# huangjuite/form

Measured on AMD Instinct MI355X. Metric: scans/sec + Mpts/sec scan-to-submap ICP (128-beam); ATE delta vs reference, higher is better.
Workload: dtype fp32 points / fp64 map, residuals and normal equations; 1 GPU; c4: 128x2048 organized scan stream (262144 pts/scan), register_scan, smoothing mode (ConstraintManager default); parallelism=replicas x1, prefill=90, pipelined_extraction=True

## Files before the change

__graft_entry__.py:

```python
from __future__ import annotations

import os
import subprocess
import sys

ROOT = os.path.dirname(os.path.abspath(__file__))


def build() -> None:
    jobs = str(min(8, os.cpu_count() or 4))
    subprocess.check_call(["make", "-s", "-j", jobs, "-C", os.path.join(ROOT, "form_amd", "csrc")])
    subprocess.check_call(["make", "-s", "-C", os.path.join(ROOT, "oracle")])
    subprocess.check_call(["make", "-s", "-C", os.path.join(ROOT, "tests", "cpp")])
    if os.path.exists(os.path.join(ROOT, "tests", "cpp", "extract_plan.mk")):
        subprocess.check_call(["make", "-s", "-C", os.path.join(ROOT, "tests", "cpp"), "-f", "extract_plan.mk"])
    if os.path.exists(os.path.join(ROOT, "tests", "cpp", "carve_host.mk")):
        subprocess.check_call(["make", "-s", "-C", os.path.join(ROOT, "tests", "cpp"), "-f", "carve_host.mk"])
    if os.path.exists(os.path.join(ROOT, "tests", "cpp", "probe_host.mk")):
        subprocess.check_call(["make", "-s", "-C", os.path.join(ROOT, "tests", "cpp"), "-f", "probe_host.mk"])
    if os.path.exists(os.path.join(ROOT, "tests", "cpp", "scan_check.mk")):
        subprocess.check_call(["make", "-s", "-C", os.path.join(ROOT, "tests", "cpp"), "-f", "scan_check.mk"])
    if os.path.exists(os.path.join(ROOT, "tests", "cpp", "upload_host.mk")):
        subprocess.check_call(["make", "-s", "-C", os.path.join(ROOT, "tests", "cpp"), "-f", "upload_host.mk"])
    if os.path.exists(os.path.join(ROOT, "tests", "cpp", "nearest_host.mk")):
        subprocess.check_call(["make", "-s", "-C", os.path.join(ROOT, "tests", "cpp"), "-f", "nearest_host.mk"])
    if os.path.exists(os.path.join(ROOT, "tests", "cpp", "align_host.mk")):
        subprocess.check_call(["make", "-s", "-C", os.path.join(ROOT, "tests", "cpp"), "-f", "align_host.mk"])
    if os.path.exists(os.path.join(ROOT, "tests", "cpp", "store_plan.mk")):
        subprocess.check_call(["make", "-s", "-C", os.path.join(ROOT, "tests", "cpp"), "-f", "store_plan.mk"])
    sys.path.insert(0, ROOT)
    import form_amd
    from form_amd import fmx
    L = fmx.lib()
    missing = [s for s in fmx.EXPORTED if not hasattr(L, s)]
    if missing:
        raise RuntimeError(f"libfmx.so is missing symbols: {missing}")


def smoke() -> None:
    import numpy as np
    import torch

    sys.path.insert(0, ROOT)
    sys.path.insert(0, os.path.join(ROOT, "oracle"))
    import oracle_py as O

    from form_amd import fmx, synth

    assert torch.cuda.is_available(), "smoke() needs a GPU"
    scan, T, geo = synth.make_scan("tiny", 0)
    p = synth.default_params(geo)
    ref = O.extract(scan.numpy(), p)
    ctx = fmx.Context(fmx.EstimatorParams(extraction=fmx.KeypointExtractionParams(**p)))
    ctx.extract(scan.to("cuda:0"), 0)
    got = ctx.extract_download()
    ok = ref["normal_ok"]
    assert np.array_equal(got["planar_index"], ref["sel"][ok]), "planar selection differs from oracle"
    assert np.array_equal(got["point_index"], ref["point_idx"]), "point selection differs from oracle"
    dots = np.abs(np.sum(got["planar"][:, 3:] * ref["normals"][ok], 1))
    assert dots.min() > 1 - 1e-5, f"normals differ (min |dot| {dots.min()})"
    est = fmx.Context(fmx.EstimatorParams(extraction=fmx.KeypointExtractionParams(**p)))
    oest = O.Estimator(O.default_params(p))
    world = synth.World()
    for k in range(3):
        s, _, _ = synth.make_scan("tiny", k, world=world)
        est.register_scan(s.to("cuda:0"))
        Tg = est.current_pose()
        To, _, _ = oest.register_scan(s.numpy())
        assert np.abs(Tg - To).max() < 1e-6, f"scan {k}: pose differs from oracle by {np.abs(Tg - To).max()}"
    print("smoke ok:", len(got["planar_index"]), "planar,", len(got["point_index"]), "point; 3-scan registration matches oracle")


if __name__ == "__main__":
    build()
    if len(sys.argv) > 1 and sys.argv[1] == "smoke":
        smoke()
```

form_amd/csrc/fmx_api.cpp:

```cpp
#include <algorithm>
#include <atomic>
#include <cfloat>
#include <cmath>
#include <cstdlib>
#include <cstring>
#include <deque>
#include <functional>
#include <unistd.h>
#include <map>
#include <new>
#include <set>
#include <vector>

#include "fmx_api.hpp"

using namespace fmx;

namespace fmx {

int match_group_for(uint64_t nq, uint32_t K) { return (int)match_group(nq, K); }
void run_map_build(fmx_ctx* c, const std::vector<uint64_t>& scans, const double* poses34, double w, hipStream_t st) {
  ++c->warm_gen;
  g8::run_map_build(c, scans, poses34, w, st);
}
void run_match(fmx_ctx* c, const double* pose_j34, double max_dist, double min_dist_map, bool sorted,
               bool defer_scatter) {
  HostScope hs(16);
  ++c->corr_gen;
  c->m.match_group = match_group_for((uint64_t)c->n_qpl + c->n_qpt, c->K);
  if (c->m.match_group != 8) gl::run_match(c, pose_j34, max_dist, min_dist_map, sorted, defer_scatter);
  else g8::run_match(c, pose_j34, max_dist, min_dist_map, sorted, defer_scatter);
}
void run_pair_scatter(fmx_ctx* c) {
  HostScope hs(17);
  if (c->m.match_group != 8) gl::run_pair_scatter(c);
  else g8::run_pair_scatter(c);
}
void run_insert(fmx_ctx* c, uint64_t scan, uint32_t* n_inserted) {
  if (c->m.match_group != 8) gl::run_insert(c, scan, n_inserted);
  else g8::run_insert(c, scan, n_inserted);
}
void run_match_linearize(fmx_ctx* c, const double* pose_j34, double max_dist, double sigma, double* dst,
                         uint32_t* flag, uint32_t seq) {
  if (match_group_for((uint64_t)c->n_qpl + c->n_qpt, c->K) != 1)
    throw StatusError(FMX_E_STATE, "fused match + linearization needs the one-lane-per-query build");
  gl::run_match_linearize(c, pose_j34, max_dist, sigma, dst, flag, seq);
}
void match_counts_fetch(fmx_ctx* c, bool wait) {
  if (c->m.match_group != 8) gl::match_counts_fetch(c, wait);
  else g8::match_counts_fetch(c, wait);
}

static const char* kProfNames[PROF_COUNT] = {"extract_rows", "closest",   "fit",       "compact", "map_build",
                                             "match",        "pair_sort", "linearize", "insert",  "window",
                                             "match_linearize", "unpack", "moments", "deskew",
                                             "organize", "dense", "carve"};

ProfScope::ProfScope(Prof& p, int i, double by, hipStream_t s) : pr(p), id(i), bytes(by), st(s) {
  if (!pr.on) return;
  auto get = [&]() {
    hipEvent_t e;
    if (!pr.free_events.empty()) {
      e = pr.free_events.back();
      pr.free_events.pop_back();
    } else {
      FMX_HIP(hipEventCreate(&e));
    }
    return e;
  };
  a = get();
  b = get();
  FMX_HIP(hipEventRecord(a, st));
}
ProfScope::~ProfScope() {
  if (!a) return;
  (void)hipEventRecord(b, st);
  ProfPending e;
  e.id = id;
  e.a = a;
  e.b = b;
  e.bytes = bytes;
// ... 642 lines not shown
  c->spec_valid = true;
  c->spec_first = first;
  if (!first) ++c->spec_launched;
}
bool use_spec_match(fmx_ctx* c, const double* pose_j) {
  if (!c->spec_valid || std::memcmp(c->spec_pose, pose_j, sizeof(c->spec_pose)) != 0) return false;
  swap_match_set(c);
  c->spec_valid = false;
  if (!c->spec_first) ++c->spec_hits;
  c->spec_first = false;
  return true;
}

void keyscan_step(fmx_ctx* c, fmx_ctx::Est& e, uint64_t j, uint32_t nfeat);
void record_cons(fmx_ctx* c, fmx_ctx::Est& e, uint64_t j);

bool trace_on() {
  static const bool v = std::getenv("FMX_TRACE") != nullptr;
  return v;
}
#define FMX_TRACE_(...)                   \
  do {                                    \
    if (trace_on()) {                     \
      fprintf(stderr, __VA_ARGS__);       \
      fflush(stderr);                     \
    }                                     \
  } while (0)

bool lin_rows() {
  static const bool v = std::getenv("FMX_MOMENTS") == nullptr;
  return v;
}

void smooth_register(fmx_ctx* c, fmx_ctx::Est& e, uint64_t j, uint32_t nfeat, const LinF& fast, uint64_t& icp,
                     uint64_t& lm_it, uint64_t& lins, bool& inserted) {
  const fmx_params& P = c->P;
  const double sigma = P.planar_constraint_sigma;
  const std::vector<uint64_t> keys = window_keys(e);
  std::map<uint64_t, int> slot;
  for (size_t k = 0; k < keys.size(); ++k) slot[keys[k]] = (int)k;
  WinGraph g;
  g.keys = keys;
  for (auto& p : e.priors) g.priors.push_back(&p);
  for (auto& m : e.margs) g.lins.push_back(&m);
  if (!fast.keys.empty()) g.lins.push_back(&fast);
  std::vector<double> table;
  const bool mom = !lin_rows();
  const bool mom_full = mom;
  std::vector<double> momv;
  std::vector<Pose> mref;
  std::vector<const double*> mp;
  std::vector<const Pose*> mri, mrj, mxi, mxj;
  MomBatch mbatch;
  for (uint32_t it = 0; it < P.max_num_rematches; ++it) {
    ++icp;
    const Pose before = e.values.at(j);
    const bool spec_hit = use_spec_match(c, before.m);
    if (!spec_hit) run_match(c, before.m, P.max_dist_matching, P.min_dist_map, true);
    c->spec_valid = false;
    const bool mom_queued = spec_hit && c->spec_mom;
    c->spec_mom = false;
    pf_launch(c, false);
    g.pairs.clear();
    for (uint32_t k = 0; k < c->K; ++k) g.pairs.push_back({slot.at(c->map_scans[k]), slot.at(j)});
    const int K = (int)c->K;
    auto maybe_spec = [&](const std::vector<Pose>& x) {
      const Pose& xj = x[slot.at(j)];
      const double lc = g.trial_lin_change, ce = g.trial_err;
      bool last_likely = lc >= 0.0 && (lc <= 1e-5 * ce || lc <= 1e-5);
      if (last_likely) {
        double xi[6], dn = 0;
        logmap(compose(inverse(before), xj), xi);
        for (double v : xi) dn += v * v;
        last_likely = std::sqrt(dn) >= P.new_pose_threshold;
      }
      if (last_likely && it + 1 < P.max_num_rematches && std::memcmp(xj.m, before.m, sizeof(xj.m)) != 0) {
        FMX_TRACE_("  spec match\n");
        if (mom) {
          std::vector<double> ref(12 * ((size_t)K + 1));
          for (int k = 0; k < K; ++k) std::memcpy(&ref[12 * k], e.values.at(c->map_scans[k]).m, 12 * sizeof(double));
          std::memcpy(&ref[12 * (size_t)K], xj.m, 12 * sizeof(double));
          spec_match(c, xj.m, false, ref.data());
        } else {
          spec_match(c, xj.m);
        }
      }
    };
    bool launched = false, ready = false;
    int nlin = 0;
    if (mom) {
      auto lin_begin = [&](const std::vector<Pose>& x) {
        HostScope hs(10);
        if (!launched && mom_queued) {
          mref.resize((size_t)K + 1);
          for (int k = 0; k <= K; ++k) std::memcpy(mref[k].m, &c->spec_mom_ref[12 * (size_t)k], 12 * sizeof(double));
          momv.resize((size_t)std::max(K, 1) * kMomPairD);
          launched = true;
          FMX_TRACE_("scan %llu it %u: moments queued with the spec match\n", (unsigned long long)j, it);
        }
        if (!launched) {
          mref.resize((size_t)K + 1);
          table.resize(12 * ((size_t)K + 1));
          for (int k = 0; k < K; ++k) mref[k] = x[slot.at(c->map_scans[k])];
          mref[K] = x[slot.at(j)];
          for (int k = 0; k <= K; ++k) std::memcpy(&table[12 * k], mref[k].m, 12 * sizeof(double));
          momv.resize((size_t)std::max(K, 1) * kMomPairD);
          FMX_TRACE_("scan %llu it %u: moments launch K %d chunks %u\n", (unsigned long long)j, it, K, c->m.max_chunks);
          win_moments_current(c, table.data(), nullptr);
          FMX_TRACE_("  launched\n");
          launched = true;
        }
        maybe_spec(x);
        mxi.resize(K);
        mxj.resize(K);
        for (int k = 0; k < K; ++k) {
          mxi[k] = &x[slot.at(c->map_scans[k])];
          mxj[k] = &x[slot.at(j)];
        }
      };
      auto lin_end = [&](double* G) {
        HostScope hs(10);
        if (!ready) {
          FMX_TRACE_("  wait\n");
          win_finish(c, momv.data());
          FMX_TRACE_("  moments in\n");
          match_counts_fetch(c, false);
          for (int k = 0; k < K; ++k)
            if (c->m.cnt_pl[k] + c->m.cnt_pt[k] == 0)
              std::fill(&momv[(size_t)k * kMomPairD], &momv[(size_t)(k + 1) * kMomPairD], 0.0);
          mp.resize(K);
          mri.resize(K);
          mrj.assign(K, &mref[K]);
          for (int k = 0; k < K; ++k) {
            mp[k] = &momv[(size_t)k * kMomPairD];
            mri[k] = &mref[k];
          }
          HostScope hp(19);
          mom_prepare(mbatch, K, mp.data(), mri.data(), mrj.data());
          FMX_TRACE_("  prepared\n");
          ready = true;
        }
        HostScope he(18);
        mom_eval(mbatch, mxi.data(), mxj.data(), 1.0 / sigma, G);
        FMX_TRACE_("  eval\n");
      };
      set_lin(g, lin_begin, lin_end);
    } else {
      auto lin_begin = [&](const std::vector<Pose>& x) {
        table.resize(12 * ((size_t)K + 1));
        for (int k = 0; k < K; ++k) std::memcpy(&table[12 * k], x[slot.at(c->map_scans[k])].m, 12 * sizeof(double));
        std::memcpy(&table[12 * (size_t)K], x[slot.at(j)].m, 12 * sizeof(double));
        HostScope hs(10);
        win_linearize_current(c, table.data(), sigma, nullptr, nlin++ == 0 ? nullptr : c->lin);
        maybe_spec(x);
      };
      auto lin_end = [&](double* G) {
        HostScope hs(10);
        win_finish(c, G);
        match_counts_fetch(c, false);
        for (int k = 0; k < K; ++k)
          if (c->m.cnt_pl[k] + c->m.cnt_pt[k] == 0) std::fill(G + (size_t)k * kPairG, G + (size_t)(k + 1) * kPairG, 0.0);
      };
      set_lin(g, lin_begin, lin_end);
    }
    HostScope* hs_lm = new HostScope(8);
    FMX_TRACE_("scan %llu it %u: lm\n", (unsigned long long)j, it);
    const WinLMResult R = window_lm(g, window_poses(e));
    FMX_TRACE_("scan %llu it %u: lm done\n", (unsigned long long)j, it);
    delete hs_lm;
    lm_it += R.iters;
    lins += R.lins;
    const Pose after = R.x[slot.at(j)];
    double xi[6];
    logmap(compose(inverse(before), after), xi);
    double dn = 0;
    for (double v : xi) dn += v * v;
    if (std::sqrt(dn) < P.new_pose_threshold) break;
    e.values[j] = after;
  }
  record_cons(c, e, j);
  if (mom_full) {
    for (uint32_t k = 0; k < c->K; ++k)
      if (c->m.cnt_pl[k] + c->m.cnt_pt[k] > 0) {
        fmx_ctx::Est::Mom& m = e.moms[{j, c->map_scans[k]}];
        m.ref_i = mref[k];
        m.ref_j = mref[c->K];
        m.phi.assign(momv.begin() + (size_t)k * kMomPairD, momv.begin() + (size_t)(k + 1) * kMomPairD);
      }
  } else {
    win_persist(c, j);
  }
  ensure_pool_room(c, 0, c->n_qpl);
  ensure_pool_room(c, 1, c->n_qpt);
  run_insert(c, j, nullptr);
  inserted = true;
  keyscan_step(c, e, j, nfeat);
  c->ev_fork.record(c->stream);
  std::vector<uint64_t> map_scans;
  {
    std::set<uint64_t> sset;
    for (int t = 0; t < 2; ++t)
      for (auto& [s, r] : c->pool[t].ranges) sset.insert(s);
    map_scans.assign(sset.begin(), sset.end());
  }
  int spec_builds = 0;
  pf_launch(c, false);
  std::vector<WinPair> prs;
  if (mom_full) {
    for (auto& [ji, m] : e.moms) prs.push_back(WinPair{ji.second, ji.first, 0, 0, 0, 0});
  } else {
    prs = win_pairs(c);
  }
  g.lins.clear();
  for (auto& m : e.margs) g.lins.push_back(&m);
  g.pairs.clear();
  for (auto& p : prs) g.pairs.push_back({slot.at(p.i), slot.at(p.j)});
  if (!prs.empty() && !mom_full) win_set_pairs(c, prs, keys);
  auto maybe_spec_map = [&](const std::vector<Pose>& x) {
    const double lc = g.trial_lin_change, ce = g.trial_err;
    if (lc >= 0.0 && (lc <= 1e-5 * ce || lc <= 1e-5) && spec_builds < 2 && !map_scans.empty()) {
      ++spec_builds;
      std::vector<double> mpo(12 * map_scans.size());
      for (size_t k = 0; k < map_scans.size(); ++k) std::memcpy(&mpo[12 * k], x[slot.at(map_scans[k])].m, 12 * sizeof(double));
      FMX_TRACE_("  spec map (drain %d)\n", (int)e.spec_map);
      if (e.spec_map) FMX_HIP(hipStreamSynchronize(c->side));
      FMX_HIP(hipStreamWaitEvent(c->side, c->ev_fork.last(), 0));
      FMX_TRACE_("  spec map build\n");
      run_map_build(c, map_scans, mpo.data(), P.max_dist_matching, c->side);
      c->ev_join.record(c->side);
      FMX_TRACE_("  spec map queued\n");
      e.spec_map = true;
      e.spec_map_scans = map_scans;
      e.spec_map_poses = std::move(mpo);
    }
  };
  if (mom_full) {
    const size_t np = prs.size();
    mp.resize(np);
    mri.resize(np);
    mrj.resize(np);
    mxi.resize(np);
    mxj.resize(np);
    for (size_t p = 0; p < np; ++p) {
      const fmx_ctx::Est::Mom& m = e.moms.at({prs[p].j, prs[p].i});
      mp[p] = m.phi.data();
      mri[p] = &m.ref_i;
      mrj[p] = &m.ref_j;
    }
    {
      HostScope hp(19);
      mom_prepare(mbatch, (int)np, mp.data(), mri.data(), mrj.data());
    }
    g.lin_begin = nullptr;
    g.lin_end = nullptr;
    g.lin_pairs = [&, np](const std::vector<Pose>& x, double* G) {
      HostScope hs(10);
      FMX_TRACE_("  full lm lin (lin change %.3e)\n", g.trial_lin_change);
      maybe_spec_map(x);
      for (size_t p = 0; p < np; ++p) {
        mxi[p] = &x[g.pairs[p].first];
        mxj[p] = &x[g.pairs[p].second];
      }
      HostScope he(18);
      mom_eval(mbatch, mxi.data(), mxj.data(), 1.0 / sigma, G);
    };
  } else {
    auto lin_begin = [&](const std::vector<Pose>& x) {
      table.resize(12 * keys.size());
      for (size_t k = 0; k < keys.size(); ++k) std::memcpy(&table[12 * k], x[k].m, 12 * sizeof(double));
      HostScope hs(10);
// ... 241 lines not shown
    bool host_done = false;
    std::function<void()> host_first;
    if (c->dsk.on)
      host_first = [&] {
        map_inputs();
        finish();
        host_done = true;
      };
    if (pf_take(c, xyzw, n, on_dev, j, &fc, c->dsk.on ? &host_first : nullptr)) {
      if (c->dsk.on) {
        std::memcpy(dsk_xi, c->dsk.pf_twist, sizeof(dsk_xi));
        dsk_src = c->dsk.pf_src;
      }
      took_pf = true;
      if (!host_done) map_inputs();
      FMX_HIP(hipStreamWaitEvent(c->stream, c->ev_join.last(), 0));
      if (!P.disable_smoothing) {
        if (!lin_rows()) {
          std::vector<double> ref(12 * ((size_t)c->K + 1));
          for (uint32_t k = 0; k < c->K; ++k) std::memcpy(&ref[12 * k], e.values.at(c->map_scans[k]).m, 12 * sizeof(double));
          std::memcpy(&ref[12 * (size_t)c->K], e.values.at(j).m, 12 * sizeof(double));
          spec_match(c, e.values.at(j).m, true, ref.data());
        } else {
          spec_match(c, e.values.at(j).m, true);
        }
      }
      if (!host_done) finish();
    } else {
      do_extract(c, xyzw, n, j, on_dev, &fc, [&] {
        map_inputs();
        finish();
      }, c->dsk.on ? dsk_xi : nullptr, dsk_cells);
    }
  }
  std::memcpy(c->dsk.last, dsk_xi, sizeof(dsk_xi));
  c->dsk.last_src = dsk_src;
  const float4* dense_src = nullptr;
  if (dense_go) {
    if (c->dsk.on) {
      dense_src = took_pf ? c->dsk.pf_out.p : c->dsk.out.p;
    } else if (took_pf && c->pf_host) {
      DM.keep.ensure(n);
      FMX_HIP(hipMemcpyAsync(DM.keep.p, c->pf_scan.p, n * sizeof(float4), hipMemcpyDeviceToDevice, c->stream));
      dense_src = DM.keep.p;
    } else {
      dense_src = on_dev ? reinterpret_cast<const float4*>(xyzw) : c->scan.p;
    }
  }
  FMX_HIP(hipStreamWaitEvent(c->stream, c->ev_join.last(), 0));
  FMX_TRACE_("scan %llu: extracted %u + %u, map queued\n", (unsigned long long)j, fc.planar, fc.point);
  HostScope* hs_icp = new HostScope(4);
  uint64_t icp = 0, lm_it = 0, lins = 0;
  bool inserted = false;
  if (!P.disable_smoothing) {
    smooth_register(c, e, j, fc.planar + fc.point, fast, icp, lm_it, lins, inserted);
  } else {
    DeviceLM lm{c, e, P.planar_constraint_sigma};
    bool converged = false;
    Pose last_after = e.values.at(j);
    for (uint32_t it = 0; it < P.max_num_rematches; ++it) {
      ++icp;
      const Pose before = e.values.at(j);
      run_match(c, before.m, P.max_dist_matching, P.min_dist_map, false);
      pf_launch(c, false);
      int li = 0;
      const Pose after = lm.optimize(before, &li);
      lm_it += li;
      double xi[6];
      logmap(compose(inverse(before), after), xi);
      double dn = 0;
      for (double x : xi) dn += x * x;
      if (std::sqrt(dn) < P.new_pose_threshold) {
        converged = true;
        last_after = after;
        break;
      }
      e.values[j] = after;
    }
    if (converged) {
      e.values[j] = last_after;
    } else {
      int li = 0;
      e.values[j] = lm.optimize(e.values.at(j), &li);
      lm_it += li;
    }
    lins = lm.linearizations;
  }
  delete hs_icp;
  pf_launch(c, true);
  if (!inserted) {
    HostScope hs_tail(5);
    record_cons(c, e, j);
    ensure_pool_room(c, 0, c->n_qpl);
    ensure_pool_room(c, 1, c->n_qpt);
    run_insert(c, j, nullptr);
    keyscan_step(c, e, j, fc.planar + fc.point);
  }
  uint32_t dense_flag = 0;
  if (dense_go) dense_flag = dense_queue(c, dense_src, n, e.values.at(j).m, j);
  if (c->dsk.on && c->ann_ptr && !c->pf_launched) {
    double nxt[6];
    const int src = deskew_next_twist(c, nxt);
    pf_launch(c, true, nxt, src);
  }
  if (dense_go) {
    dense_finish(c, dense_flag, &DM.last);
// ... 46 lines not shown
  p->max_num_keyscans = 50;
  p->max_steps_unused_keyscan = 10;
  p->max_num_recent_scans = 10;
  p->keyscan_match_ratio = 0.1;
  p->min_dist_map = 0.1;
  p->keypoint_pool_capacity = 4u << 20;
  p->max_pairs = 1024;
  p->voxel_subdivision = 1;
}


fmx_status fmx_create(const fmx_params* p, int device, fmx_ctx** out) {
  if (!p || !out) return FMX_E_INVAL;
  *out = nullptr;
  int ndev = 0;
  if (hipGetDeviceCount(&ndev) != hipSuccess || ndev == 0) return FMX_E_HIP;
  if (device < 0 || device >= ndev) return FMX_E_INVAL;
  fmx_ctx* c = new (std::nothrow) fmx_ctx();
  if (!c) return FMX_E_OOM;
  c->P = *p;
  c->device = device;
  fmx_status st = guard(c, [&] {
    int prio_lo = 0, prio_hi = 0;
    FMX_HIP(hipDeviceGetStreamPriorityRange(&prio_lo, &prio_hi));
    FMX_HIP(hipStreamCreateWithPriority(&c->stream, hipStreamNonBlocking, prio_hi));
    FMX_HIP(hipStreamCreateWithPriority(&c->lin, hipStreamNonBlocking, prio_hi));
    {
      static std::atomic<uint32_t> ctx_seq{0};
      hipDeviceProp_t pr;
      FMX_HIP(hipGetDeviceProperties(&pr, device));
      const char* cus = std::getenv("FMX_SIDE_CUS");
      const int ncu = pr.multiProcessorCount, n = cus ? std::min(ncu, std::atoi(cus)) : std::max(1, ncu / 4);
      std::vector<uint32_t> m((ncu + 31) / 32, 0u);
      if (n <= 0) {
        std::fill(m.begin(), m.end(), 0xFFFFFFFFu);
      } else {
        const int q = (int)(ctx_seq.fetch_add(1u) % (uint32_t)std::max(1, ncu / n));
        for (int i = ncu - n * (q + 1); i < ncu - n * q; ++i) m[i / 32] |= 1u << (i % 32);
      }
      FMX_HIP(hipExtStreamCreateWithCUMask(&c->side, (uint32_t)m.size(), m.data()));
      FMX_HIP(hipExtStreamCreateWithCUMask(&c->side2, (uint32_t)m.size(), m.data()));
    }
    c->ev_fork.create();
    c->ev_join.create();
    c->ev_pf.create();
    c->ev_pf_fork.create();
    const uint64_t cap = p->keypoint_pool_capacity ? p->keypoint_pool_capacity : (4u << 20);
    c->pool[0].planar = true;
    c->pool[1].planar = false;
    c->pool[0].pos.ensure(cap);
    c->pool[0].nrm.ensure(cap);
    c->pool[1].pos.ensure(cap);
    c->store_limits = parse_store_limits(std::getenv("FMX_TEST_STORE_LIMITS"));
    for (int t = 0; t < 2; ++t) {
      const uint64_t alloc = c->pool[t].pos.cap;
      c->pool[t].limit = c->store_limits.pool ? std::min<uint64_t>(c->store_limits.pool, alloc) : alloc;
    }
  });
  if (st != FMX_OK) {
    fmx_destroy(c);
    return st;
  }
  *out = c;
  return FMX_OK;
}

fmx_ctx::~fmx_ctx() {
  for (hipStream_t s : {stream, side, side2, lin})
    if (s) (void)hipStreamSynchronize(s);
  stager.stop();
  delete est;
  comm_destroy(this);
  for (hipStream_t s : {stream, side, side2, lin})
    if (s) (void)hipStreamDestroy(s);
}

void fmx_destroy(fmx_ctx* c) {
  if (!c) return;
  (void)hipSetDevice(c->device);
  delete c;
}

const char* fmx_last_error(const fmx_ctx* c) { return c ? c->err.c_str() : "null context"; }

fmx_status fmx_extract(fmx_ctx* c, const float* xyzw, size_t n, uint64_t scan, int on_dev, fmx_feature_counts* out) {
  return guard<false>(c, [&] {
    drop_match(c);
    do_extract(c, xyzw, n, scan, on_dev, out);
  });
}

fmx_status fmx_extract_download(fmx_ctx* c, float* planar, uint32_t* planar_index, float* point,
                                uint32_t* point_index, uint8_t* planar_mask) {
  return guard(c, [&] {
    if (!c->have_queries) throw StatusError(FMX_E_STATE, "no extraction");
    FMX_HIP(hipStreamSynchronize(c->stream));
    const uint32_t npl = c->n_qpl, npt = c->n_qpt;
    if (planar) {
      std::vector<float4> a(npl), b(npl);
      FMX_HIP(hipMemcpy(a.data(), c->q.pl_pos.p, npl * sizeof(float4), hipMemcpyDeviceToHost));
      FMX_HIP(hipMemcpy(b.data(), c->q.pl_nrm.p, npl * sizeof(float4), hipMemcpyDeviceToHost));
      for (uint32_t i = 0; i < npl; ++i) {
        planar[6 * i] = a[i].x; planar[6 * i + 1] = a[i].y; planar[6 * i + 2] = a[i].z;
        planar[6 * i + 3] = b[i].x; planar[6 * i + 4] = b[i].y; planar[6 * i + 5] = b[i].z;
      }
    }
// ... 676 lines not shown
  return guard(c, [&] {
    if (!c->est || !c->est->init) throw StatusError(FMX_E_STATE, "no registered scan (fmx_register_scan)");
    if (!(voxel_width > 0)) throw StatusError(FMX_E_INVAL, "voxel width must be > 0");
    if (!n_planar || !n_point) throw StatusError(FMX_E_INVAL, "null count pointers");
    finish_tail(c);
    fmx_ctx::Est& e = *c->est;
    std::set<uint64_t> sset;
    for (int t = 0; t < 2; ++t)
      for (auto& [s, r] : c->pool[t].ranges) sset.insert(s);
    std::vector<uint64_t> scans(sset.begin(), sset.end());
    std::vector<double> poses(12 * scans.size());
    for (size_t k = 0; k < scans.size(); ++k) {
      auto it = e.values.find(scans[k]);
      if (it == e.values.end()) throw StatusError(FMX_E_STATE, "keypoints of a scan without an estimate");
      std::memcpy(&poses[12 * k], it->second.m, 12 * sizeof(double));
    }
    uint32_t cnt[2] = {0, 0};
    for (int t = 0; t < 2; ++t)
      for (uint64_t s : scans) {
        auto it = c->pool[t].ranges.find(s);
        if (it != c->pool[t].ranges.end()) cnt[t] += it->second.second;
      }
    double* outs[2] = {planar, point};
    uint64_t* sids[2] = {planar_scan, point_scan};
    uint32_t* ns[2] = {n_planar, n_point};
    for (int t = 0; t < 2; ++t) {
      if (!outs[t] && !sids[t]) {
        *ns[t] = cnt[t];
        continue;
      }
      if (*ns[t] < cnt[t]) throw StatusError(FMX_E_SIZE, "map_download: buffer smaller than the map");
      std::vector<double> xyz, nrm;
      std::vector<uint64_t> sid;
      const uint32_t m = map_snapshot(c, t, scans, poses, voxel_width, xyz, nrm, sid);
      const int stride = t == 0 ? 6 : 3;
      for (uint32_t r = 0; r < m; ++r) {
        if (outs[t]) {
          std::memcpy(outs[t] + (size_t)stride * r, &xyz[3 * (size_t)r], 3 * sizeof(double));
          if (t == 0) std::memcpy(outs[t] + (size_t)stride * r + 3, &nrm[3 * (size_t)r], 3 * sizeof(double));
        }
        if (sids[t]) sids[t][r] = sid[r];
      }
      *ns[t] = m;
    }
  });
}

fmx_status fmx_last_stats(fmx_ctx* c, uint64_t* stats, int n) {
  return guard<false>(c, [&] {
    if (!stats || n < 0) throw StatusError(FMX_E_INVAL, "null stats");
    const uint64_t store[kStatsStoreN] = {c->pool[0].n_compact, c->pool[1].n_compact, c->win.n_compact,
                                          c->win.n_grow_pl, c->win.n_grow_pt};
    for (int k = 0; k < n; ++k)
      stats[k] = k < kStatsN ? c->stats[k] : k < kStatsN + kStatsStoreN ? store[k - kStatsN] : 0;
  });
}

fmx_status fmx_match_work(fmx_ctx* c, double work[3]) {
  return guard<false>(c, [&] {
    match_counts_fetch(c);
    work[0] = (double)c->n_qpl + (double)c->n_qpt;
    work[1] = c->m.last_probes;
    work[2] = c->m.last_cands;
  });
}

fmx_status fmx_match_cert(fmx_ctx* c, uint64_t counts[2], uint8_t* certified) {
  return guard(c, [&] {
    if (!c->m.have_match) throw StatusError(FMX_E_STATE, "no match results");
    match_counts_fetch(c);
    if (counts) {
      counts[0] = c->m.cert_tot[0];
      counts[1] = c->m.cert_tot[1];
    }
    if (certified) {
      const uint32_t nq = c->n_qpl + c->n_qpt;
      std::vector<uint8_t> f(nq);
      if (nq) FMX_HIP(hipMemcpy(f.data(), c->m.m_ins.p, nq, hipMemcpyDeviceToHost));
      for (uint32_t q = 0; q < nq; ++q) certified[q] = (f[q] >> 1) & 1;
    }
  });
}

fmx_status fmx_profile_match_work(fmx_ctx* c, double out[12]) {
  return guard<false>(c, [&] {
    if (!out) throw StatusError(FMX_E_INVAL, "null output");
    prof_collect(c);
    for (int k = 0; k < 2; ++k)
      for (int i = 0; i < 6; ++i) out[6 * k + i] = c->prof.mwork[k][i];
  });
}

fmx_status fmx_corr_generation(fmx_ctx* c, uint64_t* gen) {
  return guard<false>(c, [&] {
    if (!gen) throw StatusError(FMX_E_INVAL, "null output");
    *gen = c->corr_gen;
  });
}

fmx_status fmx_profile_enable(fmx_ctx* c, int on) {
  return guard<false>(c, [&] { c->prof.on = on != 0; });
}
fmx_status fmx_profile_reset(fmx_ctx* c) {
  return guard<false>(c, [&] {
    prof_collect(c);
    for (int i = 0; i < PROF_COUNT; ++i) {
      c->prof.ms[i] = 0;
// ... 24 lines not shown
```

form_amd/csrc/fmx_internal.hpp:

```cpp
#pragma once
#include <hip/hip_runtime.h>

#include <atomic>
#include <stdint.h>

#include <algorithm>
#include <map>
#include <stdexcept>
#include <chrono>
#include <cstdio>
#include <cstdlib>
#include <functional>
#include <string>
#include <type_traits>
#include <utility>
#include <vector>

#include "fmx/fmx.h"
#include "carve_host.hpp"
#include "pair_sort_plan.hpp"
#include "probe_host.hpp"
#include "nearest_host.hpp"
#include "align_host.hpp"
#include "upload_host.hpp"
// ... 311 lines not shown
  int cur = 0;
  uint64_t cap_pl = 0, cap_pt = 0, tail_pl = 0, tail_pt = 0;
  WinSegs segs;
  bool exact_pl = false, exact_pt = false;
  uint64_t n_compact = 0, n_grow_pl = 0, n_grow_pt = 0;
  DBuf<uint32_t> meta;
  const Chunk* chunks_p = nullptr;
  const uint32_t* chunk_range_p = nullptr;
  Event meta_ev;
  bool meta_ev_pending = false;
  uint32_t nch = 0;
  int npairs = 0;
  uint64_t rows_pl = 0, rows_pt = 0;
  bool chunks_valid = false;
  DBuf<double> partials, dposes;
  DBuf<uint64_t> dbg;
  DBuf<uint32_t> pticket, dticket, dflag;
  bool pending = false;
  bool pending_mom = false;
  uint32_t pending_seq = 0, pending_grid = 0;
  hipStream_t pending_st = nullptr;
  int pending_np = 0;
  HBuf<double> hG, hM, hposes;
  HBuf<uint32_t> hmeta;
};

struct MatchSet {
  DBuf<int32_t> m_pair;
  DBuf<double> m_d2;
  DBuf<double4> m_pi, m_ni;
  DBuf<uint8_t> m_ins;
  DBuf<uint32_t> hist, hist_off;
  DBuf<uint32_t> thist;
  uint32_t thist_par = 0;
  DBuf<double> c_pl, c_pt;
  DBuf<uint32_t> pair_counts;
  DBuf<uint32_t> chunk_range;
  DBuf<Chunk> chunks;
  DBuf<uint32_t> n_chunks;
  DBuf<uint32_t> pair_base;
  DBuf<uint32_t> work;
  DBuf<uint32_t> mcnt, mticket;
  DBuf<uint32_t> ins_blk, ins_off;
  HBuf<uint32_t> h_counts, h_work;
  bool have_match = false, have_corr = false, have_qo = false;
  bool scatter_pending = false;
  bool counts_pending = false;
  size_t ld_pl = 0, ld_pt = 0;
  uint32_t max_chunks = 0, work_blocks = 0;
  uint32_t match_nb_pl = 0, match_nb = 0;
  uint32_t n_qo = 0;
  bool work_copied = false;
  int match_group = 8;
  PairScatter ps;
  uint64_t rows_pl = 0, rows_pt = 0;
  std::vector<uint32_t> cnt_pl, cnt_pt;
  double last_probes = 0, last_cands = 0;
  uint32_t ins_tot[2] = {0, 0};
  uint32_t cert_tot[2] = {0, 0};
};

struct QuerySet {
  DBuf<float4> pl_pos, pl_nrm, pt_pos;
  DBuf<uint32_t> pl_idx, pt_idx;
  DBuf<uint8_t> planar_mask;
};

struct ExLaunch {
  uint32_t seq = 0;
  const volatile uint32_t* flag = nullptr;
  const uint32_t* tot = nullptr;
  size_t max_pl = 0, max_pt = 0;
  hipStream_t st = nullptr;
};

}

constexpr int kStatsN = 14;
constexpr int kStatsStoreN = 5;

struct fmx_ctx {
  fmx_ctx() = default;
  fmx_ctx(const fmx_ctx&) = delete;
  fmx_ctx& operator=(const fmx_ctx&) = delete;
  ~fmx_ctx();

  fmx_params P{};
  int device = 0;
  hipStream_t stream = nullptr;
  hipStream_t side = nullptr;
  hipStream_t side2 = nullptr;
  hipStream_t lin = nullptr;
  fmx::EvRing ev_fork, ev_join;
  std::string err;
  fmx::Prof prof;

  fmx::DBuf<float4> scan;
  fmx::DBuf<uint32_t> sel_slots, pt_slots, row_counts, row_ok, row_off;
  fmx::DBuf<int2> closest;
  fmx::DBuf<float4> nrm_slots, blk_lo, blk_hi;
  fmx::DBuf<uint32_t> scan_scratch, dev_u32;
  size_t scan_scratch_half = 0;
  fmx::HBuf<uint32_t> h_u32;
  int rows = 0, cols = 0;

  uint64_t q_scan = 0;
// ... 164 lines not shown
  fmx::DBuf<uint32_t> m_rec;
  fmx::DBuf<uint4> m_cell;
  uint64_t warm_gen = 1;
  uint64_t warm_rec_gen = 0;
  fmx::DBuf<float> cert_b2;
  double cert_pose[12] = {};
  uint64_t cert_gen = 0;

  uint32_t K = 0;
  uint64_t corr_gen = 0;
  fmx::HBuf<double> h_corr;
  fmx::HBuf<uint32_t> h_meta;
  bool nrm_attr_set = false;
  bool lds_attr_set = false;

  fmx::DBuf<double> bpart;
  fmx::DBuf<uint32_t> ticket;
  fmx::DBuf<uint32_t> fz_tickets;
  bool fz_work_pending = false;
  fmx::DBuf<uint32_t> fz_work;
  fmx::HBuf<uint32_t> fz_h_work;
  uint32_t fz_work_blocks = 0;
  fmx::DBuf<uint32_t> mprof;
  fmx::HBuf<uint32_t> h_flag;
  uint32_t flag_seq = 0;
  struct LazyMatch {
    bool pending = false;
    double pose[12];
    double max_dist = 0.0;
  } lazy;
  fmx::HBuf<double> h_poses, h_G;
  fmx::HBuf<int32_t> h_i32;

  fmx::WinStore win;

  fmx::MatchSet spec;
  bool spec_valid = false;
  bool spec_first = false;
  bool spec_mom = false;
  std::vector<double> spec_mom_ref;
  double spec_pose[12] = {};
  uint64_t spec_launched = 0, spec_hits = 0;
  uint64_t spec_map_hits = 0, spec_map_misses = 0;

  void* comm = nullptr;
  int comm_size = 1, comm_rank = 0;
  bool comm_failed = false;
  fmx::DBuf<double> d_sum;
  fmx::HBuf<uint32_t> h_hold;

  struct Est;
  Est* est = nullptr;
  uint64_t stats[kStatsN] = {};
  uint64_t host_waits = 0;
};

namespace fmx {
struct HostTiming {
  bool on = std::getenv("FMX_HOST_TIMING") != nullptr;
  double t[20] = {0};
  uint64_t n[20] = {0};
  ~HostTiming() {
    if (!on) return;
    static const char* names[20] = {"register_scan", "stream_wait", "extract", "map_build", "icp_loop",
                                    "insert+tail", "map_host_prep", "map_launches", "fast_lm", "full_lm",
                                    "lin_callback", "marginalize", "win_launch_call", "win_wait",
                                    "pf_launch", "between_calls", "match_call", "scatter_call", "mom_eval",
                                    "mom_prepare"};
    for (int i = 0; i < 20; ++i)
      if (n[i]) fprintf(stderr, "host %-14s %10.1f us total %8llu calls %8.2f us/call\n", names[i], t[i] * 1e6,
                        (unsigned long long)n[i], t[i] * 1e6 / n[i]);
    fprintf(stderr, "host device-buffer reallocations %llu\n", (unsigned long long)dbuf_reallocs().load());
  }
};
inline HostTiming& host_timing() {
  static HostTiming h;
  return h;
}
struct MatchDiag {
  bool on = std::getenv("FMX_MATCH_DIAG") != nullptr;
  uint64_t launches = 0;
  double span = 0, p50 = 0, p90 = 0, p99 = 0, pmax = 0, f50 = 0, f90 = 0, f99 = 0, mq_all = 0, mq_slow = 0;
  uint64_t mq_hist[8] = {0};
  double walk_rounds = 0, walk_steps = 0, walk_listed = 0, waves = 0;
  double cert = 0, viol = 0, warmq = 0, cert_slow = 0, warm_slow = 0, cert_bl = 0, blocks = 0;
  double ph50[4] = {0, 0, 0, 0}, ph99[4] = {0, 0, 0, 0};
  ~MatchDiag() {
    if (!on || !launches) return;
    const double n = (double)launches;
#ifdef FMX_DIAG_PHASE
    fprintf(stderr, "match diag: phase ends after block start (p50 / p99 over blocks, us): query %.1f / %.1f, own cell "
                    "%.1f / %.1f, faces %.1f / %.1f, edges+corners %.1f / %.1f\n",
            ph50[0] / n, ph99[0] / n, ph50[1] / n, ph99[1] / n, ph50[2] / n, ph99[2] / n, ph50[3] / n, ph99[3] / n);
#endif
    if (warmq > 0)
      fprintf(stderr,
              "match diag: warm certificate: %.0f of %.0f warm queries certifiable (%.3f), %.0f certified with a "
              "changed NN (must be 0); slowest 1%% of blocks: %.3f of their warm queries; blocks all certifiable: "
              "%.3f\n",
              cert, warmq, cert / warmq, viol, warm_slow > 0 ? cert_slow / warm_slow : 0.0, cert_bl / blocks);
    if (walk_listed > 0)
      fprintf(stderr, "match diag: ring-1 list walk: %.2f rounds per wave, %.3f steps and %.3f listed cells per query\n",
              walk_rounds / waves, walk_steps / (waves * 64), walk_listed / (waves * 64));
    fprintf(stderr,
            "match diag: %llu launches; span %.1f us; block dur p50 %.1f p90 %.1f p99 %.1f max %.1f us; "
            "blocks done at 50/90/99%%: %.1f %.1f %.1f us; max query cands per block: mean %.1f, slowest 1%% %.1f\n",
// ... 229 lines not shown
```

form_amd/csrc/smoother.cpp:

```cpp
#include "smoother.hpp"

#include <immintrin.h>

#include <algorithm>
#include <cmath>
#include <cstdio>
#include <cstdlib>
#include <cstring>
#ifdef FMX_LM_PROF
#include <chrono>
#include <cstdio>
namespace fmxh {
double g_lm_prof[6];
uint64_t g_lm_n[6];
static const char* kLmProfNames[6] = {"H copy + chol_solve", "trial run (launch .. lin_end)", "accept test",
                                      "after lin_end: add_pair", "iterate prologue", "trial poses"};
struct LmProfPrint {
  ~LmProfPrint() {
    for (int i = 0; i < 6; ++i)
      if (g_lm_n[i]) fprintf(stderr, "lm %-32s %10.1f us total %8llu calls %8.2f us/call\n", kLmProfNames[i],
                             g_lm_prof[i] * 1e6, (unsigned long long)g_lm_n[i], g_lm_prof[i] * 1e6 / g_lm_n[i]);
  }
} g_lm_print;
}
// ... 395 lines not shown
    chol_back_fma(a, n, y.data(), x);
    return true;
  }
  for (int i = n - 1; i >= 0; --i) {
    const double* Ui = a + (size_t)i * n;
    double s = y[i];
    for (int k = i + 1; k < n; ++k) s -= Ui[k] * x[k];
    x[i] = s / Ui[i];
  }
  return true;
}

namespace {

struct Assembler {
  const WinGraph& g;
  DenseSys base;
  explicit Assembler(const WinGraph& gr) : g(gr) {
    base.init(g.keys);
    const int D = base.D;
    for (const PriorF* P : g.priors) {
      const double inv = 1.0 / P->sigma;
      const int s = base.slot.at(P->key);
      for (int k = 0; k < 6; ++k) base.at(6 * s + k, 6 * s + k) += inv * inv;
    }
    for (const LinF* L : g.lins) {
      const int n = 6 * (int)L->keys.size(), m = n + 1;
      std::vector<int> col(n);
      for (size_t k = 0; k < L->keys.size(); ++k)
        for (int e = 0; e < 6; ++e) col[6 * k + e] = 6 * base.slot.at(L->keys[k]) + e;
      const double* I = L->info.data();
      for (int r = 0; r < n; ++r) {
        double* row = &base.A[(size_t)col[r] * (D + 1)];
        for (int c = 0; c < n; ++c) row[col[c]] += I[(size_t)r * m + c];
      }
    }
  }
  void reset(DenseSys& S) const {
    const int D = base.D, ld = D + 1;
    auto blk = [&](int si, int sj) {
      for (int r = 0; r < 6; ++r)
        std::memcpy(&S.A[(size_t)(6 * si + r) * ld + 6 * sj], &base.A[(size_t)(6 * si + r) * ld + 6 * sj],
                    6 * sizeof(double));
    };
    for (const auto& pr : g.pairs) {
      blk(pr.first, pr.first);
      blk(pr.first, pr.second);
      blk(pr.second, pr.first);
      blk(pr.second, pr.second);
    }
    for (int r = 0; r < D; ++r) S.A[(size_t)r * ld + D] = base.A[(size_t)r * ld + D];
    std::memcpy(&S.A[(size_t)D * ld], &base.A[(size_t)D * ld], ld * sizeof(double));
  }
  double run(const std::vector<Pose>& x, DenseSys& S, std::vector<double>& G, int& lins, bool started = false) const {
    const bool split = !g.pairs.empty() && g.lin_begin;
    if (split && !started) g.lin_begin(x);
    if (S.D != base.D || S.keys != base.keys) S = base;
    else reset(S);
    G.assign(g.pairs.size() * kPairG, 0.0);
    if (!split && !g.pairs.empty()) {
      g.lin_pairs(x, G.data());
      ++lins;
    }
    const int D = S.D;
    double err = 0;
    for (const PriorF* P : g.priors) {
      double l[6];
      logmap(compose(inverse(x[S.slot.at(P->key)]), P->mean), l);
      const double inv = 1.0 / P->sigma;
      const int s = S.slot.at(P->key);
      double f = 0;
      for (int k = 0; k < 6; ++k) {
        const double b = l[k] * inv;
        S.at(6 * s + k, D) += inv * b;
        S.at(D, 6 * s + k) += inv * b;
        f += b * b;
      }
      S.at(D, D) += f;
      err += 0.5 * f;
    }
    for (const LinF* L : g.lins) {
      const int n = 6 * (int)L->keys.size(), m = n + 1;
      double d[6 * 64];
      std::vector<double> dv;
      double* dp = d;
      if (n > 6 * 64) {
        dv.resize(n);
        dp = dv.data();
      }
      for (size_t k = 0; k < L->keys.size(); ++k)
        logmap(compose(inverse(L->lin[k]), x[S.slot.at(L->keys[k])]), dp + 6 * k);
      const double* I = L->info.data();
      double dGd = 0, dg = 0;
      for (int r = 0; r < n; ++r) {
        const double* Ir = I + (size_t)r * m;
        const double sr = dot(Ir, dp, n);
        const int cr = 6 * S.slot.at(L->keys[r / 6]) + r % 6;
        const double gr = Ir[n] - sr;
        S.at(cr, D) += gr;
        S.at(D, cr) += gr;
        dGd += dp[r] * sr;
        dg += dp[r] * Ir[n];
      }
      const double f = I[(size_t)n * m + n] + (dGd - 2.0 * dg);
      S.at(D, D) += f;
      err += 0.5 * f;
    }
    if (split) {
      g.lin_end(G.data());
      ++lins;
    }
    LMP_BEGIN(3);
    for (size_t p = 0; p < g.pairs.size(); ++p) {
      S.add_pair(g.pairs[p].first, g.pairs[p].second, &G[p * kPairG]);
      err += G[p * kPairG + 91];
    }
    LMP_END(3);
    return err;
  }
};

}

WinLMResult window_lm(const WinGraph& g, const std::vector<Pose>& x0) {
  WinLMResult R;
  R.x = x0;
  const bool split = !g.pairs.empty() && g.lin_begin;
  if (split) g.lin_begin(R.x);
  const Assembler asmb(g);
  DenseSys S, Sn;
  std::vector<double> Gn;
  double err = asmb.run(R.x, S, R.G, R.lins, split);
  if (err <= 0.0) return R;
  double lambda = 1e-5;
  const int D = S.D;
  std::vector<double> gg(D), Hd((size_t)D * D), dx(D);
  auto iterate = [&]() {
    LMP_BEGIN(4);
    for (int r = 0; r < D; ++r) gg[r] = S.at(r, D);
    const double cc = S.at(D, D), oldLin = 0.5 * cc;
    LMP_END(4);
    for (;;) {
      LMP_BEGIN(0);
      for (int r = 0; r < D; ++r) {
        std::memcpy(&Hd[(size_t)r * D], &S.A[(size_t)r * (D + 1)], D * sizeof(double));
        Hd[(size_t)r * D + r] += lambda;
      }
      const bool ok = chol_solve(Hd, gg.data(), dx.data(), D);
      LMP_END(0);
      bool success = false, stop = false;
      std::vector<Pose> xn;
      double nerr = err;
      if (ok) {
        LMP_BEGIN(2);
        double dHd = 0, dg = 0;
        for (int r = 0; r < D; ++r) {
          const double h = dot(&S.A[(size_t)r * (D + 1)], dx.data(), D);
          dHd += dx[r] * h;
          dg += dx[r] * gg[r];
        }
        const double newLin = 0.5 * (dHd - 2 * dg + cc), linChange = oldLin - newLin;
        LMP_END(2);
        if (linChange >= 0) {
          LMP_BEGIN(5);
          xn.resize(R.x.size());
          for (size_t k = 0; k < R.x.size(); ++k) xn[k] = compose(R.x[k], expmap(&dx[6 * k]));
          LMP_END(5);
          LMP_BEGIN(1);
          g.trial_lin_change = linChange;
          g.trial_err = err;
          nerr = asmb.run(xn, Sn, Gn, R.lins);
          g.trial_lin_change = -1.0;
          LMP_END(1);
          const double costChange = err - nerr;
          if (linChange > DBL_EPSILON * oldLin) success = (costChange / linChange) > 1e-3;
          else success = true;
          if (std::abs(costChange) < 1e-5 * err) stop = true;
        }
      }
      if (success) {
        lambda = std::max(0.0, lambda / 10.0);
        R.x.swap(xn);
        err = nerr;
        std::swap(S, Sn);
        R.G.swap(Gn);
// ... 58 lines not shown
```

form_amd/csrc/smoother.hpp:

```cpp
#pragma once
#include <stdint.h>

#include <functional>
#include <map>
#include <vector>

#include "pose.hpp"

namespace fmxh {

constexpr int kPairG = 92;

struct PriorF {
  uint64_t key;
  Pose mean;
  double sigma;
};
struct LinF {
  std::vector<uint64_t> keys;
  std::vector<Pose> lin;
  std::vector<double> info;
};

struct WinGraph {
  std::vector<uint64_t> keys;
  std::vector<const PriorF*> priors;
  std::vector<const LinF*> lins;
  std::vector<std::pair<int, int>> pairs;
  std::function<void(const std::vector<Pose>& x, double* G)> lin_pairs;
  std::function<void(const std::vector<Pose>& x)> lin_begin;
  std::function<void(double* G)> lin_end;
  mutable double trial_lin_change = -1.0, trial_err = 0.0;
};

struct WinLMResult {
  std::vector<Pose> x;
  std::vector<double> G;
  int iters = 0;
  int lins = 0;
};

WinLMResult window_lm(const WinGraph& g, const std::vector<Pose>& x0);

struct DenseSys {
  std::vector<uint64_t> keys;
  std::map<uint64_t, int> slot;
  int D = 0;
  std::vector<double> A;
  void init(const std::vector<uint64_t>& ks);
  double& at(int r, int c) { return A[(size_t)r * (D + 1) + c]; }
  void add_pair(int si, int sj, const double* G91);
  double add_prior(const PriorF& P, const Pose& x);
  double add_linf(const LinF& L, const std::vector<Pose>& xk);
};

bool chol_solve(std::vector<double>& A, const double* g, double* x, int n);
double dot(const double* p, const double* q, int n);

bool schur_marginal(const std::vector<double>& A, int n, int nm, std::vector<double>& out);

}
```

form_amd/fmx.py:

```python
from __future__ import annotations

import ctypes as C
import math
import os
from dataclasses import dataclass, fields

import numpy as np

_HERE = os.path.dirname(os.path.abspath(__file__))
LIB_PATH = os.environ.get("FMX_LIB", os.path.join(_HERE, "libfmx.so"))
_LIB = None

FMX_OK = 0
_STATUS = {1: "FMX_E_INVAL", 2: "FMX_E_SIZE", 3: "FMX_E_OOM", 4: "FMX_E_HIP", 5: "FMX_E_STATE",
           6: "FMX_E_RANGE", 7: "FMX_E_RCCL"}


class FmxError(RuntimeError):
    def __init__(self, status: int, msg: str):
        super().__init__(f"{_STATUS.get(status, status)}: {msg}")
        self.status = status


class _ExtractParams(C.Structure):
# ... 868 lines not shown

    def dense_upload(self, points, scan=None, index=None, hits=None, misses=None) -> dict:
        pts = np.ascontiguousarray(_host(points), np.float64)
        if pts.size % 3 or (pts.ndim == 2 and pts.shape[1] != 3):
            raise ValueError("points must be (N, 3)")
        pts = pts.reshape(-1, 3)
        n = len(pts)
        keep = [pts]
        A = _VoxelInput()
        A.xyz = pts.ctypes.data if n else None
        for name, a, dt in (("scan", scan, np.uint64), ("index", index, np.uint32), ("hits", hits, np.uint32),
                            ("misses", misses, np.uint32)):
            if a is None:
                continue
            a = np.ascontiguousarray(_host(a), dt).reshape(-1)
            if len(a) != n:
                raise ValueError(f"{name} must hold one value per point ({len(a)} != {n})")
            keep.append(a)
            setattr(A, name, a.ctypes.data if n else _NO_ENTRIES.ctypes.data)
        cnt = _UploadCounts()
        self._chk(self._L.fmx_upload_voxels(self.h, C.byref(A), C.c_uint32(n), C.byref(cnt)))
        del keep
        return cnt.as_dict()

    def roll_stats(self) -> dict:
        s = np.zeros(6, np.uint64)
        self._chk(self._L.fmx_roll_stats(self.h, _p(s)))
        return dict(rolls=int(s[0]), evicted=int(s[1]), spilled=int(s[2]), last_kept=int(s[3]), last_evicted=int(s[4]),
                    last_scan=int(s[5]))

    def current_pose(self) -> np.ndarray:
        T = np.zeros(12)
        self._chk(self._L.fmx_current_pose(self.h, _p(T)))
        return T.reshape(3, 4)

    def map_download(self, voxel_width: float):
        npl, npt = C.c_uint32(0), C.c_uint32(0)
        self._chk(self._L.fmx_map_download(self.h, C.c_double(voxel_width), None, None, C.byref(npl), None, None,
                                           C.byref(npt)))
        pl = np.zeros((npl.value, 6))
        spl = np.zeros(npl.value, np.uint64)
        pt = np.zeros((npt.value, 3))
        spt = np.zeros(npt.value, np.uint64)
        self._chk(self._L.fmx_map_download(self.h, C.c_double(voxel_width), _p(pl), _p(spl), C.byref(npl), _p(pt),
                                           _p(spt), C.byref(npt)))
        return {"planar": (pl[:npl.value, :3].copy(), pl[:npl.value, 3:].copy(), spl[:npl.value]),
                "point": (pt[:npt.value], None, spt[:npt.value])}

    def last_stats(self) -> dict:
        keys = ["icp_iters", "lm_iters", "matched_planar", "matched_point", "map_planar", "map_point",
                "linearizations", "map_scans", "host_waits", "spec_matches", "spec_hits", "spec_map",
                "pipelined", "window_poses",
                "pool_compactions_planar", "pool_compactions_point", "win_compactions", "win_growths_plane",
                "win_growths_point"]
        s = np.zeros(len(keys), np.uint64)
        self._chk(self._L.fmx_last_stats(self.h, _p(s), C.c_int(len(keys))))
        return {k: int(v) for k, v in zip(keys, s)}

    def match_work(self) -> dict:
        w = np.zeros(3)
        self._chk(self._L.fmx_match_work(self.h, _p(w)))
        return dict(queries=float(w[0]), probes=float(w[1]), candidates=float(w[2]))

    def moments(self, ref_i, ref_j) -> np.ndarray:
        ri = np.ascontiguousarray(ref_i, np.float64).reshape(-1, 12)
        rj = np.ascontiguousarray(ref_j, np.float64).reshape(-1, 12)
        out = np.zeros((max(self.K, 1), 272))
        self._chk(self._L.fmx_moments(self.h, _p(ri), _p(rj), _p(out)))
        return out[:self.K]

    def match_cert(self, per_query: bool = False):
        cnt = np.zeros(2, np.uint64)
        flags = np.zeros(self.n_planar + self.n_point if per_query else 0, np.uint8)
        self._chk(self._L.fmx_match_cert(self.h, _p(cnt), _p(flags) if per_query else None))
        out = dict(certified=int(cnt[0]), warm=int(cnt[1]))
        if per_query:
            out["flags"] = flags
        return out

    def profile_match_work(self) -> dict:
        w = np.zeros(12)
        self._chk(self._L.fmx_profile_match_work(self.h, _p(w)))
        return {k: dict(launches=w[6 * i], queries=w[6 * i + 1], probes=w[6 * i + 2], candidates=w[6 * i + 3],
                        certified=w[6 * i + 4], warm=w[6 * i + 5])
                for i, k in enumerate(("cold", "warm"))}

    def corr_generation(self) -> int:
        g = C.c_uint64()
        self._chk(self._L.fmx_corr_generation(self.h, C.byref(g)))
        return int(g.value)

    def profile(self, on: bool = True):
        self._chk(self._L.fmx_profile_enable(self.h, C.c_int(int(on))))

    def profile_reset(self):
        self._chk(self._L.fmx_profile_reset(self.h))

    def profile_read(self) -> dict:
        n = self._L.fmx_profile_count()
        for name, flag in ((b"carve", "_carve"), (b"dense", "_dense")):
            if not getattr(self, flag, False) and self._L.fmx_profile_name(n - 1) == name:
                n -= 1
        ms = np.zeros(n)
        la = np.zeros(n, np.uint64)
        by = np.zeros(n)
        self._chk(self._L.fmx_profile_read(self.h, _p(ms), _p(la), _p(by), C.c_int(n)))
        return {self._L.fmx_profile_name(k).decode(): dict(ms=float(ms[k]), launches=int(la[k]), bytes=float(by[k]))
# ... 419 lines not shown
```

Baseline: 1137 scans/s.

## Seed full-window LM with Gram blocks kept from the last ICP linearization

During the scan ICP loop, the first linearization's per-pair Gram blocks, pose table and map-scan list are saved together with the correspondence generation. When the full-window smoothing LM starts, the saved blocks (plus cached older pair blocks) seed its first assembly if the correspondences and poses are bit-identical. This skips one GPU linearization launch and its wait. The change adds host copies and a validity check, a test env override, and a stats counter.

```diff
diff --git a/__graft_entry__.py b/__graft_entry__.py
--- a/__graft_entry__.py
+++ b/__graft_entry__.py
@@ -28,6 +28,8 @@
         subprocess.check_call(["make", "-s", "-C", os.path.join(ROOT, "tests", "cpp"), "-f", "align_host.mk"])
     if os.path.exists(os.path.join(ROOT, "tests", "cpp", "store_plan.mk")):
         subprocess.check_call(["make", "-s", "-C", os.path.join(ROOT, "tests", "cpp"), "-f", "store_plan.mk"])
+    if os.path.exists(os.path.join(ROOT, "tests", "cpp", "test_smoother_seed.mk")):
+        subprocess.check_call(["make", "-s", "-C", os.path.join(ROOT, "tests", "cpp"), "-f", "test_smoother_seed.mk"])
     sys.path.insert(0, ROOT)
     import form_amd
     from form_amd import fmx
diff --git a/form_amd/csrc/fmx_api.cpp b/form_amd/csrc/fmx_api.cpp
--- a/form_amd/csrc/fmx_api.cpp
+++ b/form_amd/csrc/fmx_api.cpp
@@ -26,7 +26,7 @@
 void run_match(fmx_ctx* c, const double* pose_j34, double max_dist, double min_dist_map, bool sorted,
                bool defer_scatter) {
   HostScope hs(16);
-  ++c->corr_gen;
+  c->m.gen = ++c->corr_gen;
   c->m.match_group = match_group_for((uint64_t)c->n_qpl + c->n_qpt, c->K);
   if (c->m.match_group != 8) gl::run_match(c, pose_j34, max_dist, min_dist_map, sorted, defer_scatter);
   else g8::run_match(c, pose_j34, max_dist, min_dist_map, sorted, defer_scatter);
@@ -775,8 +775,15 @@
   std::vector<const double*> mp;
   std::vector<const Pose*> mri, mrj, mxi, mxj;
   MomBatch mbatch;
+  struct {
+    bool valid = false;
+    std::vector<double> G, table;
+    std::vector<uint64_t> map_scans;
+    uint64_t gen = 0;
+  } kept;
   for (uint32_t it = 0; it < P.max_num_rematches; ++it) {
     ++icp;
+    kept.valid = false;
     const Pose before = e.values.at(j);
     const bool spec_hit = use_spec_match(c, before.m);
     if (!spec_hit) run_match(c, before.m, P.max_dist_matching, P.min_dist_map, true);
@@ -874,6 +881,7 @@
         for (int k = 0; k < K; ++k) std::memcpy(&table[12 * k], x[slot.at(c->map_scans[k])].m, 12 * sizeof(double));
         std::memcpy(&table[12 * (size_t)K], x[slot.at(j)].m, 12 * sizeof(double));
         HostScope hs(10);
+        if (nlin == 0) kept.gen = c->m.gen;
         win_linearize_current(c, table.data(), sigma, nullptr, nlin++ == 0 ? nullptr : c->lin);
         maybe_spec(x);
       };
@@ -883,6 +891,12 @@
         match_counts_fetch(c, false);
         for (int k = 0; k < K; ++k)
           if (c->m.cnt_pl[k] + c->m.cnt_pt[k] == 0) std::fill(G + (size_t)k * kPairG, G + (size_t)(k + 1) * kPairG, 0.0);
+        if (nlin == 1) {
+          kept.G.assign(G, G + (size_t)K * kPairG);
+          kept.table = table;
+          kept.map_scans.assign(c->map_scans.begin(), c->map_scans.begin() + K);
+          kept.valid = true;
+        }
       };
       set_lin(g, lin_begin, lin_end);
     }
@@ -902,6 +916,7 @@
     e.values[j] = after;
   }
   record_cons(c, e, j);
+  const uint64_t persisted_gen = c->m.gen;
   if (mom_full) {
     for (uint32_t k = 0; k < c->K; ++k)
       if (c->m.cnt_pl[k] + c->m.cnt_pt[k] > 0) {
@@ -939,6 +954,34 @@
   g.pairs.clear();
   for (auto& p : prs) g.pairs.push_back({slot.at(p.i), slot.at(p.j)});
   if (!prs.empty() && !mom_full) win_set_pairs(c, prs, keys);
+  std::vector<double> seed;
+  if (!mom_full && !prs.empty() && !c->test_full_lm_launch && kept.valid && kept.gen == persisted_gen) {
+    const size_t Kk = kept.map_scans.size();
+    bool ok = std::memcmp(&kept.table[12 * Kk], e.values.at(j).m, 12 * sizeof(double)) == 0;
+    std::map<uint64_t, size_t> kslot;
+    for (size_t k = 0; k < Kk && ok; ++k) {
+      auto v = e.values.find(kept.map_scans[k]);
+      ok = v != e.values.end() && std::memcmp(&kept.table[12 * k], v->second.m, 12 * sizeof(double)) == 0;
+      kslot[kept.map_scans[k]] = k;
+    }
+    if (ok) seed.resize(prs.size() * kPairG);
+    for (size_t p = 0; p < prs.size() && ok; ++p) {
+      const double* src = nullptr;
+      if (prs[p].j == j) {
+        auto k = kslot.find(prs[p].i);
+        if (k != kslot.end()) src = &kept.G[k->second * kPairG];
+      } else {
+        auto gc = e.gcache.find({prs[p].j, prs[p].i});
+        if (gc != e.gcache.end() && gc->second.size() == (size_t)kPairG) src = gc->second.data();
+      }
+      if (src) std::memcpy(&seed[p * kPairG], src, kPairG * sizeof(double));
+      else ok = false;
+    }
+    if (ok) {
+      g.seed_G = seed.data();
+      c->full_lm_seeded = 1;
+    }
+  }
   auto maybe_spec_map = [&](const std::vector<Pose>& x) {
     const double lc = g.trial_lin_change, ce = g.trial_err;
     if (lc >= 0.0 && (lc <= 1e-5 * ce || lc <= 1e-5) && spec_builds < 2 && !map_scans.empty()) {
@@ -1286,6 +1329,7 @@
   HostScope* hs_icp = new HostScope(4);
   uint64_t icp = 0, lm_it = 0, lins = 0;
   bool inserted = false;
+  c->full_lm_seeded = 0;
   if (!P.disable_smoothing) {
     smooth_register(c, e, j, fc.planar + fc.point, fast, icp, lm_it, lins, inserted);
   } else {
@@ -1438,6 +1482,8 @@
     c->pool[0].nrm.ensure(cap);
     c->pool[1].pos.ensure(cap);
     c->store_limits = parse_store_limits(std::getenv("FMX_TEST_STORE_LIMITS"));
+    const char* full_launch = std::getenv("FMX_TEST_FULL_LM_LAUNCH");
+    c->test_full_lm_launch = full_launch && full_launch[0] == '1';
     for (int t = 0; t < 2; ++t) {
       const uint64_t alloc = c->pool[t].pos.cap;
       c->pool[t].limit = c->store_limits.pool ? std::min<uint64_t>(c->store_limits.pool, alloc) : alloc;
@@ -2220,7 +2266,10 @@
     const uint64_t store[kStatsStoreN] = {c->pool[0].n_compact, c->pool[1].n_compact, c->win.n_compact,
                                           c->win.n_grow_pl, c->win.n_grow_pt};
     for (int k = 0; k < n; ++k)
-      stats[k] = k < kStatsN ? c->stats[k] : k < kStatsN + kStatsStoreN ? store[k - kStatsN] : 0;
+      stats[k] = k < kStatsN                  ? c->stats[k]
+                 : k < kStatsN + kStatsStoreN ? store[k - kStatsN]
+                 : k == kStatsN + kStatsStoreN ? c->full_lm_seeded
+                                               : 0;
   });
 }
 
diff --git a/form_amd/csrc/fmx_internal.hpp b/form_amd/csrc/fmx_internal.hpp
--- a/form_amd/csrc/fmx_internal.hpp
+++ b/form_amd/csrc/fmx_internal.hpp
@@ -387,6 +387,7 @@
   uint32_t n_qo = 0;
   bool work_copied = false;
   int match_group = 8;
+  uint64_t gen = 0;
   PairScatter ps;
   uint64_t rows_pl = 0, rows_pt = 0;
   std::vector<uint32_t> cnt_pl, cnt_pt;
@@ -657,6 +658,8 @@
   struct Est;
   Est* est = nullptr;
   uint64_t stats[kStatsN] = {};
+  uint64_t full_lm_seeded = 0;
+  bool test_full_lm_launch = false;
   uint64_t host_waits = 0;
 };
 
diff --git a/form_amd/csrc/smoother.cpp b/form_amd/csrc/smoother.cpp
--- a/form_amd/csrc/smoother.cpp
+++ b/form_amd/csrc/smoother.cpp
@@ -471,13 +471,16 @@
     for (int r = 0; r < D; ++r) S.A[(size_t)r * ld + D] = base.A[(size_t)r * ld + D];
     std::memcpy(&S.A[(size_t)D * ld], &base.A[(size_t)D * ld], ld * sizeof(double));
   }
-  double run(const std::vector<Pose>& x, DenseSys& S, std::vector<double>& G, int& lins, bool started = false) const {
-    const bool split = !g.pairs.empty() && g.lin_begin;
+  double run(const std::vector<Pose>& x, DenseSys& S, std::vector<double>& G, int& lins, bool started = false,
+             const double* seed = nullptr) const {
+    if (g.pairs.empty()) seed = nullptr;
+    const bool split = !g.pairs.empty() && g.lin_begin && !seed;
     if (split && !started) g.lin_begin(x);
     if (S.D != base.D || S.keys != base.keys) S = base;
     else reset(S);
-    G.assign(g.pairs.size() * kPairG, 0.0);
-    if (!split && !g.pairs.empty()) {
+    if (seed) G.assign(seed, seed + g.pairs.size() * kPairG);
+    else G.assign(g.pairs.size() * kPairG, 0.0);
+    if (!split && !seed && !g.pairs.empty()) {
       g.lin_pairs(x, G.data());
       ++lins;
     }
@@ -544,12 +547,13 @@
 WinLMResult window_lm(const WinGraph& g, const std::vector<Pose>& x0) {
   WinLMResult R;
   R.x = x0;
-  const bool split = !g.pairs.empty() && g.lin_begin;
+  const double* seed = g.pairs.empty() ? nullptr : g.seed_G;
+  const bool split = !g.pairs.empty() && g.lin_begin && !seed;
   if (split) g.lin_begin(R.x);
   const Assembler asmb(g);
   DenseSys S, Sn;
   std::vector<double> Gn;
-  double err = asmb.run(R.x, S, R.G, R.lins, split);
+  double err = asmb.run(R.x, S, R.G, R.lins, split, seed);
   if (err <= 0.0) return R;
   double lambda = 1e-5;
   const int D = S.D;
diff --git a/form_amd/csrc/smoother.hpp b/form_amd/csrc/smoother.hpp
--- a/form_amd/csrc/smoother.hpp
+++ b/form_amd/csrc/smoother.hpp
@@ -30,6 +30,7 @@
   std::function<void(const std::vector<Pose>& x, double* G)> lin_pairs;
   std::function<void(const std::vector<Pose>& x)> lin_begin;
   std::function<void(double* G)> lin_end;
+  const double* seed_G = nullptr;
   mutable double trial_lin_change = -1.0, trial_err = 0.0;
 };
 
diff --git a/form_amd/fmx.py b/form_amd/fmx.py
--- a/form_amd/fmx.py
+++ b/form_amd/fmx.py
@@ -944,7 +944,8 @@
                 "linearizations", "map_scans", "host_waits", "spec_matches", "spec_hits", "spec_map",
                 "pipelined", "window_poses",
                 "pool_compactions_planar", "pool_compactions_point", "win_compactions", "win_growths_plane",
-                "win_growths_point"]
+                "win_growths_point",
+                "full_lm_seeded"]
         s = np.zeros(len(keys), np.uint64)
         self._chk(self._L.fmx_last_stats(self.h, _p(s), C.c_int(len(keys))))
         return {k: int(v) for k, v in zip(keys, s)}
```

Result: faster. 1175 scans/s (median of 5 runs) (+3.4%).
